# alibaba/euler

Measured on NVIDIA H100. Metric: sampled_edges_per_sec, higher is better.
Workload: dtype u64 ids / f32 weights+features (f64 CDF compare)

## Files before the change

### euler_b200/csrc/capi.cu

```cuda
#include <stdio.h>
#include <stdlib.h>
#include <string.h>

#include <algorithm>
#include <map>
#include <mutex>
#include <string>

#include "internal.h"

namespace eu {

__global__ void k_seed(EuRngState* rs, int n, unsigned long long seed0, const unsigned long long* seeds) {
  const int e = blockIdx.x * blockDim.x + threadIdx.x;
  if (e >= n) return;
  const unsigned long long seed = seeds ? seeds[e] : seed0 + (unsigned long long)e;
  EuRngState* r = rs + e;
  unsigned long long x = seed % 2147483647ull;
  r->x = x == 0 ? 1u : (uint32_t)x;
  r->x_prev = r->x;
  r->draws = 0;
  r->calls = 0;
  r->blocks_done = 0;
  r->key = seed * 0x9E3779B97F4A7C15ull;
}

template <typename T>
static int regrow(T** p, int64_t count) {
  if (*p) cudaFree(*p);
  *p = nullptr;
  void* q = nullptr;
  size_t bytes = (size_t)(count > 0 ? count : 1) * sizeof(T);
  cudaError_t e = cudaMalloc(&q, bytes);
  if (e != cudaSuccess) { set_error("cudaMalloc(%zu) -> %s", bytes, cudaGetErrorString(e)); return EU_ERR_CUDA; }
  *p = (T*)q;
  return EU_OK;
}

int refuse_growth_in_capture(eu_ctx* c, const char* what) {
  cudaStreamCaptureStatus st = cudaStreamCaptureStatusNone;
  if (cudaStreamIsCapturing(c->stream, &st) == cudaSuccess && st != cudaStreamCaptureStatusNone) {
    set_error("%s must grow while the ctx stream is being captured: run the op once (or call eu_ctx_reserve) before the capture", what);
    return EU_ERR_STATE;
  }
  cudaGetLastError();
  return EU_OK;
}

int ctx_reserve(eu_ctx* c, int64_t rows, int64_t table_slots) {
  int rc;
  if ((table_slots > c->tab_set_slots || rows > c->cap_rows) && (rc = refuse_growth_in_capture(c, "the sampling scratch"))) return rc;
  if (table_slots > c->tab_set_slots) {
    EU_CUDA(cudaStreamSynchronize(c->stream));
    const int64_t slots = table_slots + 64;
    if ((rc = regrow(&c->d_dedup, 2 * slots))) return rc;
    c->tab_set_slots = slots;
    for (int64_t off = 0; off < 2 * slots; off += (int64_t)1 << 20) {
      int64_t n = std::min<int64_t>((int64_t)1 << 20, 2 * slots - off);
      EU_CUDA(cudaMemset2DAsync(&c->d_dedup[off].key, sizeof(HashSlot), 0x00, 8, (size_t)n, c->stream));
      EU_CUDA(cudaMemset2DAsync(&c->d_dedup[off].row, sizeof(HashSlot), 0xFF, 8, (size_t)n, c->stream));
    }
  }
  if (rows <= c->cap_rows) return EU_OK;
  EU_CUDA(cudaStreamSynchronize(c->stream));
  if ((rc = regrow(&c->d_first, rows))) return rc;
  if ((rc = regrow(&c->d_rowof, rows))) return rc;
  if ((rc = regrow(&c->d_elig, rows))) return rc;
  if ((rc = regrow(&c->d_state, rows))) return rc;
  if ((rc = regrow(&c->d_emask, rows / 32 + 2))) return rc;
  if ((rc = regrow(&c->d_woff, rows / 32 + 2))) return rc;
  if ((rc = regrow(&c->d_blkpre, rows / 256 + 66))) return rc;
  if ((rc = regrow(&c->d_blkmul, rows / 256 + 66))) return rc;
  if ((rc = regrow(&c->d_live, rows))) return rc;
  if ((rc = regrow(&c->d_dup, rows))) return rc;
  if (!c->d_nlive && (rc = regrow(&c->d_nlive, 4))) return rc;
  if ((rc = regrow(&c->d_front[0], rows))) return rc;
  if ((rc = regrow(&c->d_front[1], rows))) return rc;
  c->cap_rows = rows;
  return EU_OK;
}

int ctx_misc(eu_ctx* c, int64_t bytes) {
  if (bytes <= c->misc_bytes) return EU_OK;
  if (int rc0 = refuse_growth_in_capture(c, "the op scratch")) return rc0;
  EU_CUDA(cudaStreamSynchronize(c->stream));
  char* p = (char*)c->d_misc;
  int rc = regrow(&p, bytes);
  c->d_misc = p;
  if (rc) { c->misc_bytes = 0; return rc; }
  c->misc_bytes = bytes;
  return EU_OK;
}

int agg_reserve(eu_ctx* c, int64_t rows, int64_t table_slots) {
  if (rows <= c->agg_rows && table_slots <= c->agg_slots) return EU_OK;
  int rc;
  if ((rc = refuse_growth_in_capture(c, "the aggregation scratch"))) return rc;
  EU_CUDA(cudaStreamSynchronize(c->stream));
  if (table_slots > c->agg_slots) {
    c->agg_slots = 0;
    if ((rc = regrow(&c->d_agg_tab, table_slots))) return rc;
    EU_CUDA(cudaMemsetAsync(c->d_agg_tab, 0, sizeof(unsigned long long) * (size_t)table_slots, c->stream));
    c->agg_slots = table_slots;
  }
  if (rows > c->agg_rows) {
    c->agg_rows = 0;
    if ((rc = regrow(&c->d_agg_src, rows))) return rc;
    if ((rc = regrow(&c->d_agg_rep, rows))) return rc;
    if ((rc = regrow(&c->d_agg_slot, rows))) return rc;
    if (!c->d_agg_nrep && (rc = regrow(&c->d_agg_nrep, 1))) return rc;
    c->agg_rows = rows;
  }
  return EU_OK;
}

static std::mutex g_default_mu;
static eu_graph* g_default_graph = nullptr;
static eu_ctx* g_default_ctx = nullptr;

}

using namespace eu;

extern "C" {

int eu_ctx_create(eu_graph* g, eu_rng_kind rng, uint64_t seed, void* stream, eu_ctx** out) {
  if (!g || !out || (rng != EU_RNG_MINSTD && rng != EU_RNG_PHILOX)) { set_error("eu_ctx_create: bad argument"); return EU_ERR_INVALID; }
  EU_CUDA(cudaSetDevice(g->device));
  eu_ctx* c = new eu_ctx();
  c->g = g; c->rng = rng; c->seed = seed; c->stream = (cudaStream_t)stream;
  cudaError_t e = cudaMalloc(&c->d_rng, sizeof(EuRngState));
  if (e != cudaSuccess) { set_error("cudaMalloc rng -> %s", cudaGetErrorString(e)); delete c; return EU_ERR_CUDA; }
  k_seed<<<1, 64, 0, c->stream>>>(c->d_rng, 1, seed, nullptr);
  g_launches++;
  *out = c;
  return EU_OK;
}

int eu_ctx_destroy(eu_ctx* c) {
  if (!c) return EU_OK;
  cudaSetDevice(c->g->device);
  cudaStreamSynchronize(c->stream);
  cudaFree(c->d_rng); cudaFree(c->d_dedup); cudaFree(c->d_first); cudaFree(c->d_rowof);
  cudaFree(c->d_elig); cudaFree(c->d_state); cudaFree(c->d_emask); cudaFree(c->d_woff); cudaFree(c->d_blkpre); cudaFree(c->d_blkmul); cudaFree(c->d_live); cudaFree(c->d_dup); cudaFree(c->d_nlive); cudaFree(c->d_front[0]); cudaFree(c->d_front[1]);
  cudaFree(c->d_misc); cudaFree(c->d_stage); cudaFree(c->d_walkv);
  cudaFree(c->d_agg_tab); cudaFree(c->d_agg_src); cudaFree(c->d_agg_rep); cudaFree(c->d_agg_slot); cudaFree(c->d_agg_nrep);
  for (int i = 0; i < 2; ++i) { if (c->aux[i]) cudaStreamDestroy(c->aux[i]); if (c->ev_join[i]) cudaEventDestroy(c->ev_join[i]); }
  if (c->ev_fork) cudaEventDestroy(c->ev_fork);
  if (c->h_pin) cudaFreeHost(c->h_pin);
  delete c;
  return EU_OK;
}

int eu_ctx_set_stream(eu_ctx* c, void* stream) {
  if (!c) { set_error("null ctx"); return EU_ERR_INVALID; }
  c->stream = (cudaStream_t)stream;
  return EU_OK;
}

int eu_ctx_seed(eu_ctx* c, uint64_t seed) {
  if (!c) { set_error("null ctx"); return EU_ERR_INVALID; }
  EU_CUDA(cudaSetDevice(c->g->device));
  c->seed = seed;
  k_seed<<<1, 64, 0, c->stream>>>(c->d_rng, c->n_eng, seed, nullptr);
  EU_LAUNCHED();
  return EU_OK;
}

int eu_ctx_set_engines(eu_ctx* c, int32_t n, const uint64_t* seeds) {
  if (!c || n < 1 || n > 64) { set_error("eu_ctx_set_engines: 1..64 engines"); return EU_ERR_INVALID; }
  EU_CUDA(cudaSetDevice(c->g->device));
  EU_CUDA(cudaStreamSynchronize(c->stream));
  EuRngState* r = nullptr;
  EU_CUDA(cudaMalloc(&r, sizeof(EuRngState) * n));
  unsigned long long* d_seeds = nullptr;
  if (seeds) {
    EU_CUDA(cudaMalloc(&d_seeds, sizeof(unsigned long long) * n));
    EU_CUDA(cudaMemcpy(d_seeds, seeds, sizeof(unsigned long long) * n, cudaMemcpyHostToDevice));
    c->seed = seeds[0];
  }
  cudaFree(c->d_rng);
  c->d_rng = r;
  c->n_eng = n;
  k_seed<<<1, 64, 0, c->stream>>>(c->d_rng, n, c->seed, d_seeds);
  EU_LAUNCHED();
  EU_CUDA(cudaStreamSynchronize(c->stream));
  if (d_seeds) cudaFree(d_seeds);
  return EU_OK;
}

int eu_ctx_reserve(eu_ctx* c, int64_t max_rows) {
  if (!c || max_rows < 0) { set_error("eu_ctx_reserve: bad argument"); return EU_ERR_INVALID; }
  EU_CUDA(cudaSetDevice(c->g->device));
  const int nb = c->n_eng;
  int rc = ctx_reserve(c, max_rows + 256 * nb, 4 * max_rows + 65 * nb);
  if (rc) return rc;
  return ctx_misc(c, 256 + 4 * max_rows);
}

int eu_ctx_sync(eu_ctx* c) {
  if (!c) { set_error("null ctx"); return EU_ERR_INVALID; }
  EU_CUDA(cudaSetDevice(c->g->device));
  EU_CUDA(cudaStreamSynchronize(c->stream));
  return EU_OK;
}

int eu_ctx_draws(eu_ctx* c, uint64_t* draws) {
  if (!c || !draws) { set_error("eu_ctx_draws: bad argument"); return EU_ERR_INVALID; }
  EU_CUDA(cudaSetDevice(c->g->device));
  EuRngState h;
  EU_CUDA(cudaMemcpyAsync(&h, c->d_rng, sizeof(h), cudaMemcpyDeviceToHost, c->stream));
  EU_CUDA(cudaStreamSynchronize(c->stream));
  *draws = h.draws;
  return EU_OK;
}

int eu_ctx_profile(eu_ctx* c, int enable) {
  if (!c) { set_error("null ctx"); return EU_ERR_INVALID; }
  c->prof = enable != 0;
  return EU_OK;
}

int eu_ctx_profile_read(eu_ctx* c, char* buf, int64_t cap) {
  if (!c || !buf || cap <= 0) { set_error("eu_ctx_profile_read: bad argument"); return EU_ERR_INVALID; }
  EU_CUDA(cudaSetDevice(c->g->device));
  EU_CUDA(cudaStreamSynchronize(c->stream));
  std::map<std::pair<std::string, int64_t>, std::pair<int64_t, double>> agg;
  for (auto& r : c->prof_recs) {
    float ms = 0.f;
    cudaEventElapsedTime(&ms, r.e0, r.e1);
    auto& a = agg[std::make_pair(std::string(r.name), r.rows)];
    a.first += 1; a.second += ms;
    cudaEventDestroy(r.e0); cudaEventDestroy(r.e1);
  }
  c->prof_recs.clear();
  std::string out;
  char line[256];
  for (auto& kv : agg) {
    snprintf(line, sizeof(line), "%s,%lld,%lld,%.6f\n", kv.first.first.c_str(), (long long)kv.first.second,
             (long long)kv.second.first, kv.second.second);
    out += line;
  }
  if ((int64_t)out.size() + 1 > cap) { set_error("profile buffer too small"); return EU_ERR_INVALID; }
  memcpy(buf, out.c_str(), out.size() + 1);
  return EU_OK;
}

eu_graph* eu_default_graph(void) { std::lock_guard<std::mutex> l(g_default_mu); return g_default_graph; }
eu_ctx* eu_default_ctx(void) { std::lock_guard<std::mutex> l(g_default_mu); return g_default_ctx; }

int eu_set_default_graph(eu_graph* g, eu_rng_kind rng, uint64_t seed) {
  std::lock_guard<std::mutex> l(g_default_mu);
  if (g_default_ctx) { eu_ctx_destroy(g_default_ctx); g_default_ctx = nullptr; }
  g_default_graph = g;
  if (!g) return EU_OK;
  return eu_ctx_create(g, rng, seed, nullptr, &g_default_ctx);
}

bool InitQueryProxy(const char* conf) {
  if (!conf) return false;
  std::map<std::string, std::string> kv;
  std::string s(conf);
  size_t pos = 0;
  int items = 0;
  while (pos <= s.size()) {
    size_t end = s.find(';', pos);
    if (end == std::string::npos) end = s.size();
    std::string item = s.substr(pos, end - pos);
    pos = end + 1;
    if (item.empty()) continue;
    size_t eq = item.find('=');
    if (eq == std::string::npos || item.find('=', eq + 1) != std::string::npos) return false;
    kv[item.substr(0, eq)] = item.substr(eq + 1);
    ++items;
  }
  if (items == 0) return false;
  std::string mode = kv.count("mode") ? kv["mode"] : "local";
  if (mode != "local") {
    fprintf(stderr, "[euler_b200] ERROR InitQueryProxy: mode=%s is not on this path (only mode=local; sharding is eu_* over NCCL)\n", mode.c_str());
    return true;
  }
  int device = kv.count("device") ? atoi(kv["device"].c_str()) : 0;
  uint64_t seed = kv.count("seed") ? strtoull(kv["seed"].c_str(), nullptr, 10) : 1;
  eu_rng_kind rng = (kv.count("rng") && kv["rng"] == "philox") ? EU_RNG_PHILOX : EU_RNG_MINSTD;
  eu_graph* g = nullptr;
  int rc = eu_graph_load(kv["data_path"].c_str(), 0, 1, device, &g);
  if (rc != EU_OK) {
    fprintf(stderr, "[euler_b200] ERROR InitQueryProxy: graph load failed: %s\n", eu_last_error());
    return true;
  }
  rc = eu_set_default_graph(g, rng, seed);
  if (rc != EU_OK) fprintf(stderr, "[euler_b200] ERROR InitQueryProxy: %s\n", eu_last_error());
  return true;
}

}
```

### euler_b200/csrc/internal.h

```cpp
#pragma once
#include <cuda_runtime.h>
#include <stdint.h>

#include <atomic>
#include <string>
#include <vector>

#include "../../include/euler_b200.h"
#include "common.cuh"

namespace eu {

void set_error(const char* fmt, ...);
extern std::atomic<uint64_t> g_launches;

#define EU_CUDA(call)                                                                    \
  do {                                                                                   \
    cudaError_t _e = (call);                                                             \
    if (_e != cudaSuccess) {                                                             \
      ::eu::set_error("%s:%d %s -> %s", __FILE__, __LINE__, #call, cudaGetErrorString(_e)); \
      return EU_ERR_CUDA;                                                                \
    }                                                                                    \
  } while (0)

#define EU_LAUNCHED()                                                              \
  do {                                                                             \
    ::eu::g_launches.fetch_add(1, std::memory_order_relaxed);                      \
    cudaError_t _e = cudaPeekAtLastError();                                        \
    if (_e != cudaSuccess) {                                                       \
      ::eu::set_error("%s:%d launch -> %s", __FILE__, __LINE__, cudaGetErrorString(_e)); \
      return EU_ERR_CUDA;                                                          \
    }                                                                              \
  } while (0)

inline int64_t ceil_div(int64_t a, int64_t b) { return (a + b - 1) / b; }

struct ETList {
  int32_t K;
  int32_t v[EU_MAX_ETYPES];
};

struct TypeSampler {
  int64_t n = 0;
  unsigned long long* ids = nullptr;
  float* prob = nullptr;
  int32_t* alias = nullptr;
  float fwc_sum = 0.f;
};

}

struct eu_graph {
  int device = 0;
  eu::DevGraph d{};
  std::vector<void*> allocs;
  int64_t hbm_bytes = 0;
  bool sampler_built = false;
  std::vector<eu::TypeSampler> samplers;
  std::vector<float> type_sums;
  std::vector<float> type_prob;
  std::vector<int32_t> type_alias;
  float type_fwc_sum = 0.f;
  float* d_type_prob = nullptr;
  int32_t* d_type_alias = nullptr;
  std::vector<int64_t> sampler_order;
  std::vector<std::string> edge_type_names, node_type_names;
  std::vector<std::string> dense_feature_names;
  std::vector<std::string> sparse_feature_names, binary_feature_names;
  std::vector<uint64_t> u64_slot_max;
  eu::DevEdges e{};
  bool edges_set = false;
  struct EdgeSampler { int64_t n = 0; const int64_t* order = nullptr; const float* prob = nullptr; const int32_t* alias = nullptr; float fwc_sum = 0.f; };
  std::vector<EdgeSampler> edge_samplers;
  std::vector<std::string> edge_dense_names, edge_sparse_names, edge_binary_names;
  bool labels_built = false;
  std::vector<std::string> labels;
  int32_t* d_label_ptr = nullptr;
  unsigned long long* d_label_ids = nullptr;

  template <typename T>
  int alloc(T** p, int64_t count) {
    size_t bytes = (size_t)(count > 0 ? count : 1) * sizeof(T);
    bytes = (bytes + 255) & ~(size_t)255;
    void* q = nullptr;
    cudaError_t e = cudaMalloc(&q, bytes);
    if (e != cudaSuccess) {
      eu::set_error("cudaMalloc(%zu) -> %s", bytes, cudaGetErrorString(e));
      return EU_ERR_CUDA;
    }
    allocs.push_back(q);
    hbm_bytes += (int64_t)bytes;
    *p = (T*)q;
    return EU_OK;
  }
};

struct EuRngState {
  uint32_t x;
  uint32_t x_prev;
  unsigned long long draws;
  unsigned long long calls;
  unsigned int blocks_done;
  unsigned int pad2;
  unsigned long long key;
};

struct eu_ctx {
  eu_graph* g = nullptr;
  eu_rng_kind rng = EU_RNG_MINSTD;
  uint64_t seed = 0;
  cudaStream_t stream = nullptr;
  EuRngState* d_rng = nullptr;
  int n_eng = 1;
  int64_t cap_rows = 0;
  eu::HashSlot* d_dedup = nullptr;
  int64_t tab_set_slots = 0;
  int32_t* d_first = nullptr;
  int64_t* d_rowof = nullptr;
  uint8_t* d_elig = nullptr;
  uint32_t* d_state = nullptr;
  uint32_t* d_emask = nullptr;
  uint32_t* d_woff = nullptr;
  uint32_t* d_blkpre = nullptr;
  uint32_t* d_blkmul = nullptr;
  int32_t* d_live = nullptr;
  int32_t* d_dup = nullptr;
  unsigned int* d_nlive = nullptr;
  unsigned long long* d_front[2] = {nullptr, nullptr};
  int64_t agg_rows = 0, agg_slots = 0;
  unsigned long long* d_agg_tab = nullptr;
  int32_t* d_agg_src = nullptr;
  int32_t* d_agg_rep = nullptr;
  uint32_t* d_agg_slot = nullptr;
  unsigned int* d_agg_nrep = nullptr;
  void* d_misc = nullptr;
  int64_t misc_bytes = 0;
  float* d_walkv = nullptr;
  long long walkv_cap = 0;
  cudaStream_t aux[2] = {nullptr, nullptr};
  cudaEvent_t ev_fork = nullptr, ev_join[2] = {nullptr, nullptr};
  void* h_pin = nullptr;
  int64_t pin_bytes = 0;
  void* d_stage = nullptr;
  int64_t stage_bytes = 0;
  bool prof = false;
  struct ProfRec { const char* name; int64_t rows; cudaEvent_t e0, e1; };
  std::vector<ProfRec> prof_recs;
};

struct EuProfScope {
  eu_ctx* c; size_t idx;
  EuProfScope(eu_ctx* c_, const char* name, int64_t rows) : c(c_), idx((size_t)-1) {
    if (!c->prof) return;
    eu_ctx::ProfRec r{name, rows, nullptr, nullptr};
    cudaEventCreate(&r.e0); cudaEventCreate(&r.e1);
    cudaEventRecord(r.e0, c->stream);
    c->prof_recs.push_back(r);
    idx = c->prof_recs.size() - 1;
  }
  ~EuProfScope() { if (idx != (size_t)-1) cudaEventRecord(c->prof_recs[idx].e1, c->stream); }
};

namespace eu {
static constexpr int64_t kRepeatMinRows = (int64_t)1 << 17;
int ctx_reserve(eu_ctx* c, int64_t rows, int64_t table_slots);
int64_t hop_scratch_rows(int nb, int64_t rows_b);
int64_t hop_table_slots(int nb, int64_t rows_b);
int64_t hop_table_cap(int64_t rows_b);
int ctx_misc(eu_ctx* c, int64_t bytes);
inline size_t a256(size_t b) { return (b + 255) & ~(size_t)255; }
struct EdgeOrder;
int segmented_row_sum(eu_ctx* c, const float* rows, const float* w, const EdgeOrder& o, const int32_t* row, int64_t E, int64_t n,
                      int dim, float* out);
size_t ragged_scan_bytes(int64_t M);
int sparse_entry_ptr(eu_ctx* c, const int64_t* nodes, int64_t M, int32_t fid, void* tmp, size_t tmp_bytes, int64_t* ptr);
int agg_reserve(eu_ctx* c, int64_t rows, int64_t table_slots);
int refuse_growth_in_capture(eu_ctx* c, const char* what);
int graph_build_sampler(eu_graph* g);
int graph_build_labels(eu_graph* g);
void graph_label_list(const std::vector<int64_t>& order, int64_t n, const int64_t* bin_ptr, const uint8_t* bin_val, int32_t S,
                      int32_t fid, std::vector<std::string>* labels, std::vector<int32_t>* row_label);
__global__ void k_advance_engine(EuRngState* rng, unsigned long long uniforms);
__global__ void k_ragged_stats(const long long* __restrict__ ptr, int64_t rows, long long* __restrict__ stats);
int agnn_dot(eu_ctx* c, const float* a, const float* b, const int32_t* ia, const int32_t* ib, int64_t E, int dim,
             const float* beta, float* dot, float* scaled);
int get_node_weight(eu_ctx* c, const int64_t* nodes, int64_t B, float* out);
int launch_state_scan(eu_ctx* c, int64_t rows, unsigned long long uniforms_per_row);
int hop(eu_ctx* c, const unsigned long long* seeds, int64_t rows, const int32_t* etypes, int32_t K,
        int32_t count, int64_t default_node, unsigned long long* eng_ids, int64_t* out_ids,
        float* out_w, int32_t* out_t, int hop_index, bool pre_inserted, bool insert_next, int nb,
        const int32_t* rows_act = nullptr, bool raw = false);
}
```

### euler_b200/csrc/mp_ops.cu

```cuda
#include <stdlib.h>

#include <cooperative_groups.h>

#include <algorithm>

#include "segment.cuh"

namespace cg = cooperative_groups;

namespace eu {

__device__ __forceinline__ float4 ldg4(const float* p) { return __ldg(reinterpret_cast<const float4*>(p)); }
__device__ __forceinline__ void st4(float* p, float4 v) { *reinterpret_cast<float4*>(p) = v; }

template <bool VEC>
__global__ void __launch_bounds__(256) k_feature(DevGraph g, const unsigned long long* __restrict__ ids,
                                                 int64_t M, int32_t dim, int G, int32_t soff, int32_t sdim,
                                                 float* __restrict__ out) {
  const int sh = 31 - __clz(G);
  const int sub = (int)(threadIdx.x & (G - 1));
  const int64_t stride = ((int64_t)gridDim.x * blockDim.x) >> sh;
  for (int64_t i = (blockIdx.x * (int64_t)blockDim.x + threadIdx.x) >> sh; i < M; i += stride) {
    const int64_t row = sdim > 0 ? lookup_row(g, ids[i]) : -1;
    const int32_t fd = sdim;
    float* o = out + i * (int64_t)dim;
    const float* f = row >= 0 ? g.feat + row * (int64_t)g.feat_dim + soff : nullptr;
    if (VEC) {
      for (int32_t d = sub * 4; d < dim; d += G * 4) {
        float4 v = make_float4(0.f, 0.f, 0.f, 0.f);
        if (f && d < fd) v = ldg4(f + d);
        st4(o + d, v);
      }
    } else {
      for (int32_t d = sub; d < dim; d += G) o[d] = (f && d < fd) ? __ldg(f + d) : 0.f;
    }
  }
}

template <bool VEC>
__global__ void __launch_bounds__(256) k_gather(const float* __restrict__ params, int64_t D,
                                                const int32_t* __restrict__ idx, int64_t E, int G,
                                                float* __restrict__ out) {
  const int64_t tid = blockIdx.x * (int64_t)blockDim.x + threadIdx.x;
  const int64_t i = tid >> (31 - __clz(G));
  const int sub = (int)(tid & (G - 1));
  if (i >= E) return;
  const float* src = params + (int64_t)__ldg(idx + i) * D;
  float* o = out + i * D;
  if (VEC) {
    for (int64_t d = sub * 4; d < D; d += G * 4) st4(o + d, ldg4(src + d));
  } else {
    for (int64_t d = sub; d < D; d += G) o[d] = __ldg(src + d);
  }
}

enum { OP_ADD = 0, OP_MAX = 1, OP_MEAN = 2 };

template <int OP, bool VEC>
__global__ void __launch_bounds__(256) k_scatter_sorted(const float* __restrict__ upd, int64_t D,
                                                        const int32_t* __restrict__ idx, int64_t E,
                                                        int64_t size, int G, const int* unsorted,
                                                        float* __restrict__ out) {
  if (*unsorted) return;
  const int64_t tid = blockIdx.x * (int64_t)blockDim.x + threadIdx.x;
  const int64_t r = tid >> (31 - __clz(G));
  const int sub = (int)(tid & (G - 1));
  if (r >= size) return;
  const int64_t b = key_lower_bound(idx, E, r), e = key_lower_bound(idx, E, r + 1);
  const float init = OP == OP_MAX ? -1e9f : 0.f;
  const float denom = __fadd_rn((float)(e - b), 1e-7f);
  float* o = out + r * D;
  if (VEC) {
    for (int64_t d = sub * 4; d < D; d += G * 4) {
      float4 acc = make_float4(init, init, init, init);
      for (int64_t k = b; k < e; ++k) {
        float4 v = ldg4(upd + k * D + d);
        if (OP == OP_MAX) {
          acc.x = v.x > acc.x ? v.x : acc.x; acc.y = v.y > acc.y ? v.y : acc.y;
          acc.z = v.z > acc.z ? v.z : acc.z; acc.w = v.w > acc.w ? v.w : acc.w;
        } else {
          acc.x = __fadd_rn(acc.x, v.x); acc.y = __fadd_rn(acc.y, v.y);
          acc.z = __fadd_rn(acc.z, v.z); acc.w = __fadd_rn(acc.w, v.w);
        }
      }
      if (OP == OP_MEAN) {
        acc.x = __fdiv_rn(acc.x, denom); acc.y = __fdiv_rn(acc.y, denom);
        acc.z = __fdiv_rn(acc.z, denom); acc.w = __fdiv_rn(acc.w, denom);
      }
      st4(o + d, acc);
    }
  } else {
    for (int64_t d = sub; d < D; d += G) {
      float acc = init;
      for (int64_t k = b; k < e; ++k) {
        float v = __ldg(upd + k * D + d);
        if (OP == OP_MAX) acc = v > acc ? v : acc; else acc = __fadd_rn(acc, v);
      }
      if (OP == OP_MEAN) acc = __fdiv_rn(acc, denom);
      o[d] = acc;
    }
  }
}

__global__ void k_fill_if(float* __restrict__ out, int64_t n, float v, const int* unsorted) {
  if (!*unsorted) return;
  int64_t i = blockIdx.x * (int64_t)blockDim.x + threadIdx.x;
  const int64_t stride = (int64_t)gridDim.x * blockDim.x;
  for (; i < n; i += stride) out[i] = v;
}

__device__ __forceinline__ void atomic_max_f32(float* addr, float v) {
  if (v != v) return;
  if (v >= 0.f) atomicMax(reinterpret_cast<int*>(addr), __float_as_int(v));
  else atomicMin(reinterpret_cast<unsigned int*>(addr), __float_as_uint(v));
}

template <int OP, bool VEC>
__global__ void __launch_bounds__(256) k_scatter_atomic(const float* __restrict__ upd, int64_t D,
                                                        const int32_t* __restrict__ idx, int64_t E, int G,
                                                        const int* unsorted, float* __restrict__ out,
                                                        float* __restrict__ cnt) {
  if (!*unsorted) return;
  const int64_t tid = blockIdx.x * (int64_t)blockDim.x + threadIdx.x;
  const int64_t i = tid >> (31 - __clz(G));
  const int sub = (int)(tid & (G - 1));
  if (i >= E) return;
  const int64_t r = __ldg(idx + i);
  float* o = out + r * D;
  const float* u = upd + i * D;
  if (OP == OP_MEAN && sub == 0) atomicAdd(cnt + r, 1.0f);
  if (VEC && OP != OP_MAX) {
    for (int64_t d = sub * 4; d < D; d += G * 4) atomicAdd(reinterpret_cast<float4*>(o + d), ldg4(u + d));
  } else {
    const int step = VEC ? 4 : 1;
    for (int64_t d = sub * step; d < D; d += G * step)
      for (int q = 0; q < step; ++q) {
        if (OP == OP_MAX) atomic_max_f32(o + d + q, __ldg(u + d + q));
        else atomicAdd(o + d + q, __ldg(u + d + q));
      }
  }
}

__global__ void k_mean_div(float* __restrict__ out, int64_t D, int64_t size, const float* __restrict__ cnt,
                           const int* unsorted) {
  if (!*unsorted) return;
  int64_t i = blockIdx.x * (int64_t)blockDim.x + threadIdx.x;
  if (i < size * D) out[i] = __fdiv_rn(out[i], __fadd_rn(cnt[i / D], 1e-7f));
}

__global__ void __launch_bounds__(256) k_sage_classify(DevGraph g, const unsigned long long* __restrict__ ids, int64_t rows,
                                                       int32_t count, unsigned long long* tab, unsigned long long mask,
                                                       int32_t* __restrict__ src, int32_t* __restrict__ reps,
                                                       uint32_t* __restrict__ rep_slot, unsigned int* n_rep) {
  const int64_t stride = (int64_t)gridDim.x * blockDim.x;
  for (int64_t r = blockIdx.x * (int64_t)blockDim.x + threadIdx.x; r < rows; r += stride) {
    const unsigned long long* seg = ids + r * count;
    unsigned long long h = 0;
    bool any = false;
#pragma unroll 4
    for (int32_t j = 0; j < count; ++j) {
      const unsigned long long id = __ldg(seg + j);
      any |= lookup_row(g, id) >= 0;
      h = mix64(h + id + 1);
    }
    if (!any) { src[r] = -1; continue; }
    const unsigned long long tag = h & 0xFFFFFFFF00000000ull;
    unsigned long long p = h & mask;
    while (true) {
      unsigned long long sl = *reinterpret_cast<volatile unsigned long long*>(tab + p);
      if (sl == 0ull) {
        sl = atomicCAS(tab + p, 0ull, tag | (unsigned long long)(r + 1));
        if (sl == 0ull) {
          src[r] = (int32_t)r;
          const cg::coalesced_group grp = cg::coalesced_threads();
          unsigned int q = 0;
          if (grp.thread_rank() == 0) q = atomicAdd(n_rep, grp.size());
          q = grp.shfl(q, 0) + grp.thread_rank();
          reps[q] = (int32_t)r;
          rep_slot[q] = (uint32_t)p;
          break;
        }
      }
      if ((sl & 0xFFFFFFFF00000000ull) == tag) {
        const int64_t o = (int64_t)(sl & 0xFFFFFFFFull) - 1;
        const unsigned long long* os = ids + o * count;
        bool same = true;
#pragma unroll 4
        for (int32_t j = 0; j < count; ++j) same &= __ldg(seg + j) == __ldg(os + j);
        if (same) { src[r] = (int32_t)o; break; }
      }
      p = (p + 1) & mask;
    }
  }
}

template <int NV, bool FULL>
__global__ void __launch_bounds__(256) k_sage_mean(DevGraph g, const unsigned long long* __restrict__ ids,
                                                   int64_t rows, const int32_t* __restrict__ list, const unsigned int* __restrict__ n_list,
                                                   int32_t count, bool mean, float* __restrict__ out) {
  const int lane = threadIdx.x & 31;
  const int32_t fd = FULL ? NV * 128 : g.feat_dim;
  const float* __restrict__ feat = g.feat + lane * 4;
  const int64_t nwarps = ((int64_t)gridDim.x * blockDim.x) >> 5;
  const int64_t n = list ? (int64_t)__ldg(n_list) : rows;
  for (int64_t q = (blockIdx.x * (int64_t)blockDim.x + threadIdx.x) >> 5; q < n; q += nwarps) {
  const int64_t r = list ? (int64_t)__ldg(list + q) : q;
  float4 acc[NV];
#pragma unroll
  for (int v = 0; v < NV; ++v) acc[v] = make_float4(0.f, 0.f, 0.f, 0.f);
  for (int32_t j0 = 0; j0 < count; j0 += 32) {
    int32_t my = -1;
    if (j0 + lane < count) my = (int32_t)lookup_row(g, __ldg(ids + r * count + j0 + lane));
    unsigned valid = __ballot_sync(0xffffffffu, my >= 0);
    while (valid) {
      float4 v[4][NV];
      int n = 0;
#pragma unroll
      for (int q = 0; q < 4; ++q) {
        if (valid) {
          const int j = __ffs(valid) - 1;
          valid &= valid - 1;
          const int32_t row = __shfl_sync(0xffffffffu, my, j);
          const float* p = feat + (int64_t)row * fd;
#pragma unroll
          for (int t = 0; t < NV; ++t) v[q][t] = (FULL || lane * 4 + t * 128 < fd) ? ldg4(p + t * 128) : make_float4(0.f, 0.f, 0.f, 0.f);
          n = q + 1;
        }
      }
#pragma unroll
      for (int q = 0; q < 4; ++q) {
        if (q < n) {
#pragma unroll
          for (int t = 0; t < NV; ++t) {
            acc[t].x = __fadd_rn(acc[t].x, v[q][t].x); acc[t].y = __fadd_rn(acc[t].y, v[q][t].y);
            acc[t].z = __fadd_rn(acc[t].z, v[q][t].z); acc[t].w = __fadd_rn(acc[t].w, v[q][t].w);
          }
        }
      }
    }
  }
  const float denom = __fadd_rn((float)count, 1e-7f);
  float* o = out + r * (int64_t)fd + lane * 4;
#pragma unroll
  for (int t = 0; t < NV; ++t) {
    float4 a = acc[t];
    if (mean) { a.x = __fdiv_rn(a.x, denom); a.y = __fdiv_rn(a.y, denom); a.z = __fdiv_rn(a.z, denom); a.w = __fdiv_rn(a.w, denom); }
    if (FULL || lane * 4 + t * 128 < fd) st4(o + t * 128, a);
  }
  }
}

__global__ void __launch_bounds__(256) k_sage_mean_generic(DevGraph g, const unsigned long long* __restrict__ ids,
                                                           int64_t rows, const int32_t* __restrict__ list, const unsigned int* __restrict__ n_list,
                                                           int32_t count, int32_t dim, bool mean, float* __restrict__ out) {
  const int lane = threadIdx.x & 31;
  const int32_t fd = g.feat_dim;
  const float denom = __fadd_rn((float)count, 1e-7f);
  const int64_t nwarps = ((int64_t)gridDim.x * blockDim.x) >> 5;
  const int64_t n = list ? (int64_t)__ldg(n_list) : rows;
  for (int64_t q = (blockIdx.x * (int64_t)blockDim.x + threadIdx.x) >> 5; q < n; q += nwarps) {
    const int64_t r = list ? (int64_t)__ldg(list + q) : q;
    for (int32_t d = lane; d < dim; d += 32) {
      float acc = 0.f;
      for (int32_t j = 0; j < count; ++j) {
        const int64_t row = lookup_row(g, __ldg(ids + r * count + j));
        acc = __fadd_rn(acc, (row >= 0 && d < fd) ? __ldg(g.feat + row * (int64_t)fd + d) : 0.f);
      }
      out[r * (int64_t)dim + d] = mean ? __fdiv_rn(acc, denom) : acc;
    }
  }
}

template <bool VEC>
__global__ void __launch_bounds__(256) k_sage_broadcast(const int32_t* __restrict__ src, int64_t rows, int32_t dim, int G,
                                                        const uint32_t* __restrict__ rep_slot, const unsigned int* __restrict__ n_rep,
                                                        unsigned long long* tab, float* out) {
  const int sh = 31 - __clz(G);
  const int sub = (int)(threadIdx.x & (G - 1));
  const int64_t gtid = blockIdx.x * (int64_t)blockDim.x + threadIdx.x;
  const int64_t nthreads = (int64_t)gridDim.x * blockDim.x;
  for (int64_t r = gtid >> sh; r < rows; r += nthreads >> sh) {
    const int64_t s = __ldg(src + r);
    if (s == r) continue;
    float* o = out + r * (int64_t)dim;
    const float* f = s >= 0 ? out + s * (int64_t)dim : nullptr;
    if (VEC) {
      for (int32_t d = sub * 4; d < dim; d += G * 4) st4(o + d, f ? ldg4(f + d) : make_float4(0.f, 0.f, 0.f, 0.f));
    } else {
      for (int32_t d = sub; d < dim; d += G) o[d] = f ? __ldg(f + d) : 0.f;
    }
  }
  const int64_t n = (int64_t)__ldg(n_rep);
  for (int64_t q = gtid; q < n; q += nthreads) tab[__ldg(rep_slot + q)] = 0ull;
}

static inline unsigned capped_grid(int64_t want_blocks, const char* env, int dflt) {
  static int cached_sage = -1, cached_feat = -1;
  int& cached = env[3] == 'S' ? cached_sage : cached_feat;
  if (cached < 0) { const char* e = getenv(env); cached = e ? std::max(0, atoi(e)) : dflt; }
  const int64_t cap = cached > 0 ? (int64_t)kSMs * cached : want_blocks;
  return (unsigned)std::max<int64_t>(1, std::min(want_blocks, cap));
}

template <int OP>
static int scatter(eu_ctx* c, const float* upd, int64_t D, const int32_t* idx, int64_t E, int64_t size,
                   float* out) {
  if (!c || D <= 0 || E < 0 || size < 0 || (E > 0 && (!upd || !idx)) || (size > 0 && !out)) {
    set_error("scatter: bad argument");
    return EU_ERR_INVALID;
  }
  EU_CUDA(cudaSetDevice(c->g->device));
  if (size == 0) return EU_OK;
  int rc = ctx_misc(c, 256 + (OP == OP_MEAN ? (int64_t)sizeof(float) * size : 0));
  if (rc) return rc;
  int* unsorted = (int*)c->d_misc;
  float* cnt = (float*)((char*)c->d_misc + 256);
  cudaStream_t s = c->stream;
  EU_CUDA(cudaMemsetAsync(unsorted, 0, sizeof(int), s));
  if (OP == OP_MEAN) EU_CUDA(cudaMemsetAsync(cnt, 0, sizeof(float) * size, s));
  const bool vec = (D % 4 == 0) && aligned16(upd) && aligned16(out);
  const int G = vec ? group_lanes(D / 4) : (D >= 32 ? 32 : 1);
  const int tb = 256;
  if (E > 1) {
    k_check_sorted<<<(unsigned)ceil_div(E, tb), tb, 0, s>>>(idx, E, unsorted);
    EU_LAUNCHED();
  }
  const unsigned gs = (unsigned)ceil_div(size * G, tb), ge = (unsigned)ceil_div((E > 0 ? E : 1) * G, tb);
  EuProfScope ps(c, "scatter(sorted+fallback)", E);
  if (vec) k_scatter_sorted<OP, true><<<gs, tb, 0, s>>>(upd, D, idx, E, size, G, unsorted, out);
  else k_scatter_sorted<OP, false><<<gs, tb, 0, s>>>(upd, D, idx, E, size, G, unsorted, out);
  EU_LAUNCHED();
  k_fill_if<<<kSMs * 4, tb, 0, s>>>(out, size * D, OP == OP_MAX ? -1e9f : 0.f, unsorted);
  EU_LAUNCHED();
  if (E > 0) {
    if (vec) k_scatter_atomic<OP, true><<<ge, tb, 0, s>>>(upd, D, idx, E, G, unsorted, out, cnt);
    else k_scatter_atomic<OP, false><<<ge, tb, 0, s>>>(upd, D, idx, E, G, unsorted, out, cnt);
    EU_LAUNCHED();
  }
  if (OP == OP_MEAN) {
    k_mean_div<<<(unsigned)ceil_div(size * D, tb), tb, 0, s>>>(out, D, size, cnt, unsorted);
    EU_LAUNCHED();
  }
  return EU_OK;
}

}

using namespace eu;

extern "C" {

int eu_get_dense_feature(eu_ctx* c, const int64_t* nodes, int64_t M, int32_t fid, int32_t dim, float* out) {
  if (!c || M < 0 || dim < 0 || (M > 0 && (!nodes || (dim > 0 && !out)))) { set_error("eu_get_dense_feature: bad argument"); return EU_ERR_INVALID; }
  EU_CUDA(cudaSetDevice(c->g->device));
  if (M == 0 || dim == 0) return EU_OK;
  const DevGraph& d = c->g->d;
  const bool have = fid >= 0 && fid < d.n_slots;
  const int32_t soff = have ? d.slot_off[fid] : 0, sdim = have ? d.slot_dim[fid] : 0;
  const bool vec = (dim % 4 == 0) && (d.feat_dim % 4 == 0) && (soff % 4 == 0) && (sdim % 4 == 0) && aligned16(out);
  const int G = vec ? group_lanes(dim / 4) : (dim >= 32 ? 32 : 1);
  const unsigned blocks = capped_grid(ceil_div(M * G, 256), "EU_FEATURE_CTAS", 0);
  EuProfScope ps(c, "k_feature", M);
  if (vec) k_feature<true><<<blocks, 256, 0, c->stream>>>(d, (const unsigned long long*)nodes, M, dim, G, soff, sdim, out);
  else k_feature<false><<<blocks, 256, 0, c->stream>>>(d, (const unsigned long long*)nodes, M, dim, G, soff, sdim, out);
  EU_LAUNCHED();
  return EU_OK;
}

int eu_gather(eu_ctx* c, const float* params, int64_t N, int64_t D, const int32_t* idx, int64_t E, float* out) {
  (void)N;
  if (!c || D <= 0 || E < 0 || (E > 0 && (!params || !idx || !out))) { set_error("eu_gather: bad argument"); return EU_ERR_INVALID; }
  EU_CUDA(cudaSetDevice(c->g->device));
  if (E == 0) return EU_OK;
  const bool vec = (D % 4 == 0) && aligned16(params) && aligned16(out);
  const int G = vec ? group_lanes(D / 4) : (D >= 32 ? 32 : 1);
  const unsigned blocks = (unsigned)ceil_div(E * G, 256);
  if (vec) k_gather<true><<<blocks, 256, 0, c->stream>>>(params, D, idx, E, G, out);
  else k_gather<false><<<blocks, 256, 0, c->stream>>>(params, D, idx, E, G, out);
  EU_LAUNCHED();
  return EU_OK;
}

int eu_scatter_add(eu_ctx* c, const float* u, int64_t D, const int32_t* idx, int64_t E, int64_t size, float* out) {
  return scatter<OP_ADD>(c, u, D, idx, E, size, out);
}
int eu_scatter_max(eu_ctx* c, const float* u, int64_t D, const int32_t* idx, int64_t E, int64_t size, float* out) {
  return scatter<OP_MAX>(c, u, D, idx, E, size, out);
}
int eu_scatter_mean(eu_ctx* c, const float* u, int64_t D, const int32_t* idx, int64_t E, int64_t size, float* out) {
  return scatter<OP_MEAN>(c, u, D, idx, E, size, out);
}

static int fanout_aggregate(eu_ctx* c, const int64_t* nbr_ids, int64_t rows, int32_t count, int32_t dim, bool mean, float* out) {
  if (!c || rows < 0 || count < 0 || dim <= 0 || (rows > 0 && (!nbr_ids || !out))) { set_error("eu_sage_mean_aggregate: bad argument"); return EU_ERR_INVALID; }
  EU_CUDA(cudaSetDevice(c->g->device));
  if (rows == 0) return EU_OK;
  cudaStream_t s = c->stream;
  const DevGraph& d = c->g->d;
  const unsigned long long* ids = (const unsigned long long*)nbr_ids;
  const bool dedup = rows >= kRepeatMinRows && rows < ((int64_t)1 << 31);
  int64_t cap = 64;
  while (cap < 2 * rows) cap <<= 1;
  if (dedup) {
    int rc = agg_reserve(c, rows, cap);
    if (rc) return rc;
    EU_CUDA(cudaMemsetAsync(c->d_agg_nrep, 0, sizeof(unsigned int), s));
    EuProfScope ps(c, "k_sage_classify", rows);
    k_sage_classify<<<capped_grid(ceil_div(rows, 256), "EU_SAGE_CTAS", 0), 256, 0, s>>>(d, ids, rows, count, c->d_agg_tab, (unsigned long long)cap - 1,
                                                                                      c->d_agg_src, c->d_agg_rep, c->d_agg_slot, c->d_agg_nrep);
    EU_LAUNCHED();
  }
  const unsigned blocks = capped_grid(ceil_div(rows * 32, 256), "EU_SAGE_CTAS", 0);
  const int32_t* reps = dedup ? c->d_agg_rep : nullptr;
  const unsigned int* nrep = c->d_agg_nrep;
  { EuProfScope ps(c, mean ? "k_sage_mean" : "k_sage_add", rows);
  const bool v4 = d.n < ((int64_t)1 << 31) && d.n_slots == 1 && dim == d.feat_dim && (dim & 3) == 0 && dim <= 1024 && aligned16(out) && aligned16(d.feat);
  if (v4 && dim == 128) k_sage_mean<1, true><<<blocks, 256, 0, s>>>(d, ids, rows, reps, nrep, count, mean, out);
  else if (v4 && dim == 256) k_sage_mean<2, true><<<blocks, 256, 0, s>>>(d, ids, rows, reps, nrep, count, mean, out);
  else if (v4 && dim <= 128) k_sage_mean<1, false><<<blocks, 256, 0, s>>>(d, ids, rows, reps, nrep, count, mean, out);
  else if (v4 && dim <= 256) k_sage_mean<2, false><<<blocks, 256, 0, s>>>(d, ids, rows, reps, nrep, count, mean, out);
  else if (v4 && dim <= 512) k_sage_mean<4, false><<<blocks, 256, 0, s>>>(d, ids, rows, reps, nrep, count, mean, out);
  else if (v4) k_sage_mean<8, false><<<blocks, 256, 0, s>>>(d, ids, rows, reps, nrep, count, mean, out);
  else k_sage_mean_generic<<<blocks, 256, 0, s>>>(d, ids, rows, reps, nrep, count, dim, mean, out); }
  EU_LAUNCHED();
  if (!dedup) return EU_OK;
  { EuProfScope ps(c, "k_sage_broadcast", rows);
    const bool vec = (dim & 3) == 0 && aligned16(out);
    const int G = vec ? group_lanes(dim / 4) : (dim >= 32 ? 32 : 1);
    const unsigned bb = capped_grid(ceil_div(rows * G, 256), "EU_SAGE_CTAS", 0);
    if (vec) k_sage_broadcast<true><<<bb, 256, 0, s>>>(c->d_agg_src, rows, dim, G, c->d_agg_slot, nrep, c->d_agg_tab, out);
    else k_sage_broadcast<false><<<bb, 256, 0, s>>>(c->d_agg_src, rows, dim, G, c->d_agg_slot, nrep, c->d_agg_tab, out); }
  EU_LAUNCHED();
  return EU_OK;
}

int eu_sage_mean_aggregate(eu_ctx* c, const int64_t* nbr_ids, int64_t rows, int32_t count, int32_t dim, float* out) {
  return fanout_aggregate(c, nbr_ids, rows, count, dim, true, out);
}
int eu_sage_add_aggregate(eu_ctx* c, const int64_t* nbr_ids, int64_t rows, int32_t count, int32_t dim, float* out) {
  return fanout_aggregate(c, nbr_ids, rows, count, dim, false, out);
}

}
```

Before: 5.505 billion.

## Fuse SAGE aggregation dedup into a tiled single kernel with shared-memory hashing

Replaces the three-kernel global dedup pipeline (classify into a global hash table, aggregate representatives, broadcast copies) with one tiled kernel. Each block resolves node rows for a tile of neighbor lists into shared memory, deduplicates identical rows with a shared hash table, sums features once per unique row and writes the result to every duplicate. This drops two launches, the global table memset and cleanup, and the read-back of output rows in broadcast. In exchange, dedup now only catches repeats within a tile, and the large shared-memory footprint may limit occupancy.

```diff
diff --git a/euler_b200/csrc/capi.cu b/euler_b200/csrc/capi.cu
--- a/euler_b200/csrc/capi.cu
+++ b/euler_b200/csrc/capi.cu
@@ -92,28 +92,6 @@
   return EU_OK;
 }
 
-int agg_reserve(eu_ctx* c, int64_t rows, int64_t table_slots) {
-  if (rows <= c->agg_rows && table_slots <= c->agg_slots) return EU_OK;
-  int rc;
-  if ((rc = refuse_growth_in_capture(c, "the aggregation scratch"))) return rc;
-  EU_CUDA(cudaStreamSynchronize(c->stream));
-  if (table_slots > c->agg_slots) {
-    c->agg_slots = 0;
-    if ((rc = regrow(&c->d_agg_tab, table_slots))) return rc;
-    EU_CUDA(cudaMemsetAsync(c->d_agg_tab, 0, sizeof(unsigned long long) * (size_t)table_slots, c->stream));
-    c->agg_slots = table_slots;
-  }
-  if (rows > c->agg_rows) {
-    c->agg_rows = 0;
-    if ((rc = regrow(&c->d_agg_src, rows))) return rc;
-    if ((rc = regrow(&c->d_agg_rep, rows))) return rc;
-    if ((rc = regrow(&c->d_agg_slot, rows))) return rc;
-    if (!c->d_agg_nrep && (rc = regrow(&c->d_agg_nrep, 1))) return rc;
-    c->agg_rows = rows;
-  }
-  return EU_OK;
-}
-
 static std::mutex g_default_mu;
 static eu_graph* g_default_graph = nullptr;
 static eu_ctx* g_default_ctx = nullptr;
@@ -144,7 +122,6 @@
   cudaFree(c->d_rng); cudaFree(c->d_dedup); cudaFree(c->d_first); cudaFree(c->d_rowof);
   cudaFree(c->d_elig); cudaFree(c->d_state); cudaFree(c->d_emask); cudaFree(c->d_woff); cudaFree(c->d_blkpre); cudaFree(c->d_blkmul); cudaFree(c->d_live); cudaFree(c->d_dup); cudaFree(c->d_nlive); cudaFree(c->d_front[0]); cudaFree(c->d_front[1]);
   cudaFree(c->d_misc); cudaFree(c->d_stage); cudaFree(c->d_walkv);
-  cudaFree(c->d_agg_tab); cudaFree(c->d_agg_src); cudaFree(c->d_agg_rep); cudaFree(c->d_agg_slot); cudaFree(c->d_agg_nrep);
   for (int i = 0; i < 2; ++i) { if (c->aux[i]) cudaStreamDestroy(c->aux[i]); if (c->ev_join[i]) cudaEventDestroy(c->ev_join[i]); }
   if (c->ev_fork) cudaEventDestroy(c->ev_fork);
   if (c->h_pin) cudaFreeHost(c->h_pin);
diff --git a/euler_b200/csrc/internal.h b/euler_b200/csrc/internal.h
--- a/euler_b200/csrc/internal.h
+++ b/euler_b200/csrc/internal.h
@@ -127,12 +127,6 @@
   int32_t* d_dup = nullptr;
   unsigned int* d_nlive = nullptr;
   unsigned long long* d_front[2] = {nullptr, nullptr};
-  int64_t agg_rows = 0, agg_slots = 0;
-  unsigned long long* d_agg_tab = nullptr;
-  int32_t* d_agg_src = nullptr;
-  int32_t* d_agg_rep = nullptr;
-  uint32_t* d_agg_slot = nullptr;
-  unsigned int* d_agg_nrep = nullptr;
   void* d_misc = nullptr;
   int64_t misc_bytes = 0;
   float* d_walkv = nullptr;
@@ -174,7 +168,6 @@
                       int dim, float* out);
 size_t ragged_scan_bytes(int64_t M);
 int sparse_entry_ptr(eu_ctx* c, const int64_t* nodes, int64_t M, int32_t fid, void* tmp, size_t tmp_bytes, int64_t* ptr);
-int agg_reserve(eu_ctx* c, int64_t rows, int64_t table_slots);
 int refuse_growth_in_capture(eu_ctx* c, const char* what);
 int graph_build_sampler(eu_graph* g);
 int graph_build_labels(eu_graph* g);
diff --git a/euler_b200/csrc/mp_ops.cu b/euler_b200/csrc/mp_ops.cu
--- a/euler_b200/csrc/mp_ops.cu
+++ b/euler_b200/csrc/mp_ops.cu
@@ -1,12 +1,9 @@
+#include <limits.h>
 #include <stdlib.h>
 
-#include <cooperative_groups.h>
-
 #include <algorithm>
 
 #include "segment.cuh"
-
-namespace cg = cooperative_groups;
 
 namespace eu {
 
@@ -148,96 +145,165 @@
   if (i < size * D) out[i] = __fdiv_rn(out[i], __fadd_rn(cnt[i / D], 1e-7f));
 }
 
-__global__ void __launch_bounds__(256) k_sage_classify(DevGraph g, const unsigned long long* __restrict__ ids, int64_t rows,
-                                                       int32_t count, unsigned long long* tab, unsigned long long mask,
-                                                       int32_t* __restrict__ src, int32_t* __restrict__ reps,
-                                                       uint32_t* __restrict__ rep_slot, unsigned int* n_rep) {
-  const int64_t stride = (int64_t)gridDim.x * blockDim.x;
-  for (int64_t r = blockIdx.x * (int64_t)blockDim.x + threadIdx.x; r < rows; r += stride) {
-    const unsigned long long* seg = ids + r * count;
-    unsigned long long h = 0;
-    bool any = false;
-#pragma unroll 4
-    for (int32_t j = 0; j < count; ++j) {
-      const unsigned long long id = __ldg(seg + j);
-      any |= lookup_row(g, id) >= 0;
-      h = mix64(h + id + 1);
-    }
-    if (!any) { src[r] = -1; continue; }
-    const unsigned long long tag = h & 0xFFFFFFFF00000000ull;
-    unsigned long long p = h & mask;
-    while (true) {
-      unsigned long long sl = *reinterpret_cast<volatile unsigned long long*>(tab + p);
-      if (sl == 0ull) {
-        sl = atomicCAS(tab + p, 0ull, tag | (unsigned long long)(r + 1));
-        if (sl == 0ull) {
-          src[r] = (int32_t)r;
-          const cg::coalesced_group grp = cg::coalesced_threads();
-          unsigned int q = 0;
-          if (grp.thread_rank() == 0) q = atomicAdd(n_rep, grp.size());
-          q = grp.shfl(q, 0) + grp.thread_rank();
-          reps[q] = (int32_t)r;
-          rep_slot[q] = (uint32_t)p;
-          break;
+template <int NV, bool FULL>
+__device__ __forceinline__ void sage_row_sum(const float* __restrict__ feat, int32_t fd, int lane, int32_t my, float4 (&acc)[NV]) {
+  unsigned valid = __ballot_sync(0xffffffffu, my >= 0);
+  while (valid) {
+    float4 v[4][NV];
+    int n = 0;
+#pragma unroll
+    for (int q = 0; q < 4; ++q) {
+      if (valid) {
+        const int j = __ffs(valid) - 1;
+        valid &= valid - 1;
+        const int32_t row = __shfl_sync(0xffffffffu, my, j);
+        const float* p = feat + (int64_t)row * fd;
+#pragma unroll
+        for (int t = 0; t < NV; ++t) v[q][t] = (FULL || lane * 4 + t * 128 < fd) ? ldg4(p + t * 128) : make_float4(0.f, 0.f, 0.f, 0.f);
+        n = q + 1;
+      }
+    }
+#pragma unroll
+    for (int q = 0; q < 4; ++q) {
+      if (q < n) {
+#pragma unroll
+        for (int t = 0; t < NV; ++t) {
+          acc[t].x = __fadd_rn(acc[t].x, v[q][t].x); acc[t].y = __fadd_rn(acc[t].y, v[q][t].y);
+          acc[t].z = __fadd_rn(acc[t].z, v[q][t].z); acc[t].w = __fadd_rn(acc[t].w, v[q][t].w);
         }
       }
-      if ((sl & 0xFFFFFFFF00000000ull) == tag) {
-        const int64_t o = (int64_t)(sl & 0xFFFFFFFFull) - 1;
-        const unsigned long long* os = ids + o * count;
-        bool same = true;
-#pragma unroll 4
-        for (int32_t j = 0; j < count; ++j) same &= __ldg(seg + j) == __ldg(os + j);
-        if (same) { src[r] = (int32_t)o; break; }
-      }
-      p = (p + 1) & mask;
-    }
+    }
+  }
+}
+
+static constexpr int kTileMaxRows = 256;
+static constexpr int kTileIds = 8192;
+template <int NV, bool FULL> constexpr int tile_threads() { return NV == 1 || (NV == 2 && FULL) ? 512 : 256; }
+
+template <int NV, bool FULL>
+__global__ void __launch_bounds__(tile_threads<NV, FULL>(), tile_threads<NV, FULL>() == 512 ? 2 : 1) k_sage_mean_tiled(DevGraph g, const unsigned long long* __restrict__ ids, int64_t rows,
+                                                         int32_t count, int T, bool mean, float* __restrict__ out) {
+  __shared__ int32_t s_row[kTileIds];
+  __shared__ unsigned long long s_tab[2 * kTileMaxRows];
+  __shared__ int32_t s_first[2 * kTileMaxRows];
+  __shared__ int32_t s_src[kTileMaxRows];
+  __shared__ int32_t s_list[kTileMaxRows];
+  __shared__ int s_n;
+  const int tid = threadIdx.x, lane = tid & 31;
+  const int32_t fd = FULL ? NV * 128 : g.feat_dim;
+  const float* __restrict__ feat = g.feat + lane * 4;
+  const float denom = __fadd_rn((float)count, 1e-7f);
+  const int nslot = 2 * T;
+  const int64_t tiles = (rows + T - 1) / T;
+  for (int64_t tile = blockIdx.x; tile < tiles; tile += gridDim.x) {
+    const int64_t r0 = tile * T;
+    const int n = (int)min((int64_t)T, rows - r0);
+    const unsigned long long* tids = ids + r0 * count;
+    for (int k0 = 0; k0 < n * count; k0 += 8 * blockDim.x) {
+      unsigned long long v[8];
+#pragma unroll
+      for (int u = 0; u < 8; ++u) { const int k = k0 + u * blockDim.x + tid; v[u] = k < n * count ? __ldg(tids + k) : 0ull; }
+#pragma unroll
+      for (int u = 0; u < 8; ++u) {
+        const int k = k0 + u * blockDim.x + tid;
+        if (k < n * count) s_row[k] = (int32_t)lookup_row(g, v[u]);
+      }
+    }
+    for (int k = tid; k < nslot; k += blockDim.x) {
+      s_tab[k] = 0ull;
+      s_first[k] = INT_MAX;
+    }
+    if (tid == 0) s_n = 0;
+    __syncthreads();
+    int slot = -1;
+    if (tid < n) {
+      const int32_t* seg = s_row + tid * count;
+      unsigned long long h = 0;
+      bool any = false;
+      for (int32_t j = 0; j < count; ++j) {
+        any |= seg[j] >= 0;
+        h = mix64(h + (unsigned long long)(uint32_t)(seg[j] + 1) + 1);
+      }
+      if (any) {
+        const unsigned long long tag = h & 0xFFFFFFFF00000000ull;
+        int p = (int)(h & (unsigned long long)(nslot - 1));
+        while (true) {
+          const unsigned long long sl = atomicCAS(s_tab + p, 0ull, tag | (unsigned long long)(tid + 1));
+          if (sl == 0ull) break;
+          if ((sl & 0xFFFFFFFF00000000ull) == tag) {
+            const int32_t* os = s_row + ((int)(sl & 0xFFFFFFFFull) - 1) * count;
+            bool same = true;
+            for (int32_t j = 0; j < count; ++j) same &= seg[j] == os[j];
+            if (same) break;
+          }
+          p = (p + 1) & (nslot - 1);
+        }
+        slot = p;
+        atomicMin(s_first + slot, tid);
+      }
+    }
+    __syncthreads();
+    const int first = slot >= 0 ? s_first[slot] : -1;
+    if (tid < n) s_src[tid] = first;
+    const unsigned lead = __ballot_sync(0xffffffffu, tid < n && first == tid);
+    int at = 0;
+    if (lane == 0 && lead) at = atomicAdd(&s_n, __popc(lead));
+    at = __shfl_sync(0xffffffffu, at, 0);
+    if (tid < n && first == tid) s_list[at + __popc(lead & ((1u << lane) - 1))] = tid;
+    const unsigned zero = __ballot_sync(0xffffffffu, tid < n && slot < 0);
+    for (unsigned m = zero; m; m &= m - 1) {
+      float* o = out + (r0 + (tid & ~31) + __ffs(m) - 1) * (int64_t)fd + lane * 4;
+#pragma unroll
+      for (int t = 0; t < NV; ++t)
+        if (FULL || lane * 4 + t * 128 < fd) st4(o + t * 128, make_float4(0.f, 0.f, 0.f, 0.f));
+    }
+    __syncthreads();
+    const int groups = s_n;
+    for (int q = tid >> 5; q < groups; q += blockDim.x >> 5) {
+      const int e = s_list[q];
+      float4 acc[NV];
+#pragma unroll
+      for (int v = 0; v < NV; ++v) acc[v] = make_float4(0.f, 0.f, 0.f, 0.f);
+      for (int32_t j0 = 0; j0 < count; j0 += 32)
+        sage_row_sum<NV, FULL>(feat, fd, lane, j0 + lane < count ? s_row[e * count + j0 + lane] : -1, acc);
+      if (mean) {
+#pragma unroll
+        for (int t = 0; t < NV; ++t) {
+          acc[t].x = __fdiv_rn(acc[t].x, denom); acc[t].y = __fdiv_rn(acc[t].y, denom);
+          acc[t].z = __fdiv_rn(acc[t].z, denom); acc[t].w = __fdiv_rn(acc[t].w, denom);
+        }
+      }
+      for (int k0 = 0; k0 < n; k0 += 32) {
+        unsigned m = __ballot_sync(0xffffffffu, k0 + lane < n && s_src[k0 + lane] == e);
+        while (m) {
+          const int i = __ffs(m) - 1;
+          m &= m - 1;
+          float* o = out + (r0 + k0 + i) * (int64_t)fd + lane * 4;
+#pragma unroll
+          for (int t = 0; t < NV; ++t)
+            if (FULL || lane * 4 + t * 128 < fd) st4(o + t * 128, acc[t]);
+        }
+      }
+    }
+    __syncthreads();
   }
 }
 
 template <int NV, bool FULL>
 __global__ void __launch_bounds__(256) k_sage_mean(DevGraph g, const unsigned long long* __restrict__ ids,
-                                                   int64_t rows, const int32_t* __restrict__ list, const unsigned int* __restrict__ n_list,
-                                                   int32_t count, bool mean, float* __restrict__ out) {
+                                                   int64_t rows, int32_t count, bool mean, float* __restrict__ out) {
   const int lane = threadIdx.x & 31;
   const int32_t fd = FULL ? NV * 128 : g.feat_dim;
   const float* __restrict__ feat = g.feat + lane * 4;
   const int64_t nwarps = ((int64_t)gridDim.x * blockDim.x) >> 5;
-  const int64_t n = list ? (int64_t)__ldg(n_list) : rows;
-  for (int64_t q = (blockIdx.x * (int64_t)blockDim.x + threadIdx.x) >> 5; q < n; q += nwarps) {
-  const int64_t r = list ? (int64_t)__ldg(list + q) : q;
+  for (int64_t r = (blockIdx.x * (int64_t)blockDim.x + threadIdx.x) >> 5; r < rows; r += nwarps) {
   float4 acc[NV];
 #pragma unroll
   for (int v = 0; v < NV; ++v) acc[v] = make_float4(0.f, 0.f, 0.f, 0.f);
   for (int32_t j0 = 0; j0 < count; j0 += 32) {
     int32_t my = -1;
     if (j0 + lane < count) my = (int32_t)lookup_row(g, __ldg(ids + r * count + j0 + lane));
-    unsigned valid = __ballot_sync(0xffffffffu, my >= 0);
-    while (valid) {
-      float4 v[4][NV];
-      int n = 0;
-#pragma unroll
-      for (int q = 0; q < 4; ++q) {
-        if (valid) {
-          const int j = __ffs(valid) - 1;
-          valid &= valid - 1;
-          const int32_t row = __shfl_sync(0xffffffffu, my, j);
-          const float* p = feat + (int64_t)row * fd;
-#pragma unroll
-          for (int t = 0; t < NV; ++t) v[q][t] = (FULL || lane * 4 + t * 128 < fd) ? ldg4(p + t * 128) : make_float4(0.f, 0.f, 0.f, 0.f);
-          n = q + 1;
-        }
-      }
-#pragma unroll
-      for (int q = 0; q < 4; ++q) {
-        if (q < n) {
-#pragma unroll
-          for (int t = 0; t < NV; ++t) {
-            acc[t].x = __fadd_rn(acc[t].x, v[q][t].x); acc[t].y = __fadd_rn(acc[t].y, v[q][t].y);
-            acc[t].z = __fadd_rn(acc[t].z, v[q][t].z); acc[t].w = __fadd_rn(acc[t].w, v[q][t].w);
-          }
-        }
-      }
-    }
+    sage_row_sum<NV, FULL>(feat, fd, lane, my, acc);
   }
   const float denom = __fadd_rn((float)count, 1e-7f);
   float* o = out + r * (int64_t)fd + lane * 4;
@@ -251,15 +317,12 @@
 }
 
 __global__ void __launch_bounds__(256) k_sage_mean_generic(DevGraph g, const unsigned long long* __restrict__ ids,
-                                                           int64_t rows, const int32_t* __restrict__ list, const unsigned int* __restrict__ n_list,
-                                                           int32_t count, int32_t dim, bool mean, float* __restrict__ out) {
+                                                           int64_t rows, int32_t count, int32_t dim, bool mean, float* __restrict__ out) {
   const int lane = threadIdx.x & 31;
   const int32_t fd = g.feat_dim;
   const float denom = __fadd_rn((float)count, 1e-7f);
   const int64_t nwarps = ((int64_t)gridDim.x * blockDim.x) >> 5;
-  const int64_t n = list ? (int64_t)__ldg(n_list) : rows;
-  for (int64_t q = (blockIdx.x * (int64_t)blockDim.x + threadIdx.x) >> 5; q < n; q += nwarps) {
-    const int64_t r = list ? (int64_t)__ldg(list + q) : q;
+  for (int64_t r = (blockIdx.x * (int64_t)blockDim.x + threadIdx.x) >> 5; r < rows; r += nwarps) {
     for (int32_t d = lane; d < dim; d += 32) {
       float acc = 0.f;
       for (int32_t j = 0; j < count; ++j) {
@@ -269,29 +332,6 @@
       out[r * (int64_t)dim + d] = mean ? __fdiv_rn(acc, denom) : acc;
     }
   }
-}
-
-template <bool VEC>
-__global__ void __launch_bounds__(256) k_sage_broadcast(const int32_t* __restrict__ src, int64_t rows, int32_t dim, int G,
-                                                        const uint32_t* __restrict__ rep_slot, const unsigned int* __restrict__ n_rep,
-                                                        unsigned long long* tab, float* out) {
-  const int sh = 31 - __clz(G);
-  const int sub = (int)(threadIdx.x & (G - 1));
-  const int64_t gtid = blockIdx.x * (int64_t)blockDim.x + threadIdx.x;
-  const int64_t nthreads = (int64_t)gridDim.x * blockDim.x;
-  for (int64_t r = gtid >> sh; r < rows; r += nthreads >> sh) {
-    const int64_t s = __ldg(src + r);
-    if (s == r) continue;
-    float* o = out + r * (int64_t)dim;
-    const float* f = s >= 0 ? out + s * (int64_t)dim : nullptr;
-    if (VEC) {
-      for (int32_t d = sub * 4; d < dim; d += G * 4) st4(o + d, f ? ldg4(f + d) : make_float4(0.f, 0.f, 0.f, 0.f));
-    } else {
-      for (int32_t d = sub; d < dim; d += G) o[d] = f ? __ldg(f + d) : 0.f;
-    }
-  }
-  const int64_t n = (int64_t)__ldg(n_rep);
-  for (int64_t q = gtid; q < n; q += nthreads) tab[__ldg(rep_slot + q)] = 0ull;
 }
 
 static inline unsigned capped_grid(int64_t want_blocks, const char* env, int dflt) {
@@ -398,38 +438,28 @@
   cudaStream_t s = c->stream;
   const DevGraph& d = c->g->d;
   const unsigned long long* ids = (const unsigned long long*)nbr_ids;
-  const bool dedup = rows >= kRepeatMinRows && rows < ((int64_t)1 << 31);
-  int64_t cap = 64;
-  while (cap < 2 * rows) cap <<= 1;
-  if (dedup) {
-    int rc = agg_reserve(c, rows, cap);
-    if (rc) return rc;
-    EU_CUDA(cudaMemsetAsync(c->d_agg_nrep, 0, sizeof(unsigned int), s));
-    EuProfScope ps(c, "k_sage_classify", rows);
-    k_sage_classify<<<capped_grid(ceil_div(rows, 256), "EU_SAGE_CTAS", 0), 256, 0, s>>>(d, ids, rows, count, c->d_agg_tab, (unsigned long long)cap - 1,
-                                                                                      c->d_agg_src, c->d_agg_rep, c->d_agg_slot, c->d_agg_nrep);
-    EU_LAUNCHED();
-  }
-  const unsigned blocks = capped_grid(ceil_div(rows * 32, 256), "EU_SAGE_CTAS", 0);
-  const int32_t* reps = dedup ? c->d_agg_rep : nullptr;
-  const unsigned int* nrep = c->d_agg_nrep;
-  { EuProfScope ps(c, mean ? "k_sage_mean" : "k_sage_add", rows);
+  EuProfScope ps(c, mean ? "k_sage_mean" : "k_sage_add", rows);
   const bool v4 = d.n < ((int64_t)1 << 31) && d.n_slots == 1 && dim == d.feat_dim && (dim & 3) == 0 && dim <= 1024 && aligned16(out) && aligned16(d.feat);
-  if (v4 && dim == 128) k_sage_mean<1, true><<<blocks, 256, 0, s>>>(d, ids, rows, reps, nrep, count, mean, out);
-  else if (v4 && dim == 256) k_sage_mean<2, true><<<blocks, 256, 0, s>>>(d, ids, rows, reps, nrep, count, mean, out);
-  else if (v4 && dim <= 128) k_sage_mean<1, false><<<blocks, 256, 0, s>>>(d, ids, rows, reps, nrep, count, mean, out);
-  else if (v4 && dim <= 256) k_sage_mean<2, false><<<blocks, 256, 0, s>>>(d, ids, rows, reps, nrep, count, mean, out);
-  else if (v4 && dim <= 512) k_sage_mean<4, false><<<blocks, 256, 0, s>>>(d, ids, rows, reps, nrep, count, mean, out);
-  else if (v4) k_sage_mean<8, false><<<blocks, 256, 0, s>>>(d, ids, rows, reps, nrep, count, mean, out);
-  else k_sage_mean_generic<<<blocks, 256, 0, s>>>(d, ids, rows, reps, nrep, count, dim, mean, out); }
-  EU_LAUNCHED();
-  if (!dedup) return EU_OK;
-  { EuProfScope ps(c, "k_sage_broadcast", rows);
-    const bool vec = (dim & 3) == 0 && aligned16(out);
-    const int G = vec ? group_lanes(dim / 4) : (dim >= 32 ? 32 : 1);
-    const unsigned bb = capped_grid(ceil_div(rows * G, 256), "EU_SAGE_CTAS", 0);
-    if (vec) k_sage_broadcast<true><<<bb, 256, 0, s>>>(c->d_agg_src, rows, dim, G, c->d_agg_slot, nrep, c->d_agg_tab, out);
-    else k_sage_broadcast<false><<<bb, 256, 0, s>>>(c->d_agg_src, rows, dim, G, c->d_agg_slot, nrep, c->d_agg_tab, out); }
+  if (v4 && (int64_t)count * 32 <= kTileIds) {
+    int T = kTileMaxRows;
+    while (T > 32 && ((int64_t)T * count > kTileIds || ceil_div(rows, T) < (int64_t)kSMs * 2)) T >>= 1;
+    const unsigned blocks = capped_grid(ceil_div(rows, T), "EU_SAGE_CTAS", 0);
+    if (dim == 128) k_sage_mean_tiled<1, true><<<blocks, tile_threads<1, true>(), 0, s>>>(d, ids, rows, count, T, mean, out);
+    else if (dim == 256) k_sage_mean_tiled<2, true><<<blocks, tile_threads<2, true>(), 0, s>>>(d, ids, rows, count, T, mean, out);
+    else if (dim <= 128) k_sage_mean_tiled<1, false><<<blocks, tile_threads<1, false>(), 0, s>>>(d, ids, rows, count, T, mean, out);
+    else if (dim <= 256) k_sage_mean_tiled<2, false><<<blocks, tile_threads<2, false>(), 0, s>>>(d, ids, rows, count, T, mean, out);
+    else if (dim <= 512) k_sage_mean_tiled<4, false><<<blocks, tile_threads<4, false>(), 0, s>>>(d, ids, rows, count, T, mean, out);
+    else k_sage_mean_tiled<8, false><<<blocks, tile_threads<8, false>(), 0, s>>>(d, ids, rows, count, T, mean, out);
+  } else {
+    const unsigned blocks = capped_grid(ceil_div(rows * 32, 256), "EU_SAGE_CTAS", 0);
+    if (v4 && dim == 128) k_sage_mean<1, true><<<blocks, 256, 0, s>>>(d, ids, rows, count, mean, out);
+    else if (v4 && dim == 256) k_sage_mean<2, true><<<blocks, 256, 0, s>>>(d, ids, rows, count, mean, out);
+    else if (v4 && dim <= 128) k_sage_mean<1, false><<<blocks, 256, 0, s>>>(d, ids, rows, count, mean, out);
+    else if (v4 && dim <= 256) k_sage_mean<2, false><<<blocks, 256, 0, s>>>(d, ids, rows, count, mean, out);
+    else if (v4 && dim <= 512) k_sage_mean<4, false><<<blocks, 256, 0, s>>>(d, ids, rows, count, mean, out);
+    else if (v4) k_sage_mean<8, false><<<blocks, 256, 0, s>>>(d, ids, rows, count, mean, out);
+    else k_sage_mean_generic<<<blocks, 256, 0, s>>>(d, ids, rows, count, dim, mean, out);
+  }
   EU_LAUNCHED();
   return EU_OK;
 }
```

Measured after the change: 5.658 billion, median of 6. 1.03x the previous value.
